# jhhung/kISS

Measured on AMD Instinct MI355X. Metric: bases/sec suffix_sort (chm13v2.0-size synthetic, k=256), higher is better.
Workload: dtype u8; 1 GPU; suffix_sort genome-like synthetic n=3117292070 k=256 (stand-in for chm13v2.0.fa, BASELINE.json configs[1]); PARALLEL_SORTING; text resident in HBM, SA left in HBM; n=3117292070, k=256, seed=2, parallelism=single GPU, lms=905939973, lms_rounds=9, tied_after_round0_item_rounds=184319413, big_segment_item_rounds=72866550, workspace_bytes=80356032300, induce_passes=47

## Files before the change

### include/kiss_hip.h

```cpp
#ifndef KISS_HIP_H
#define KISS_HIP_H

#include <stddef.h>
#include <stdint.h>

#ifdef __cplusplus
extern "C" {
#endif

#define KISS_HIP_VERSION 103

typedef enum kiss_hip_status {
    KISS_HIP_OK = 0,
    KISS_HIP_E_INVALID = -1,
    KISS_HIP_E_NO_DEVICE = -2,
    KISS_HIP_E_HIP = -3,
    KISS_HIP_E_NOMEM = -4,
    KISS_HIP_E_UNSUPPORTED = -5,
    KISS_HIP_E_INTERNAL = -6,
    KISS_HIP_E_IO = -7,
    KISS_HIP_E_DEEP = -8
} kiss_hip_status;

#define KISS_HIP_ALGO_PARALLEL_SORTING 0
// ... 2 lines not shown
#define KISS_HIP_MAX_N 4294963200ull

typedef struct kiss_hip_ctx kiss_hip_ctx;

typedef struct kiss_hip_stats {
    uint64_t n;
    uint64_t m;
    uint32_t k;
    uint32_t depth;
    uint32_t lms_rounds;
    uint32_t induce_passes;
    uint64_t near_end;
    uint64_t sort_item_rounds;
    uint64_t big_item_rounds;
    float ms_total;
    float ms_pack;
    float ms_classify;
    float ms_lms_sort;
    float ms_place;
    float ms_induce;
    float ms_kernel[16];
    uint64_t launches_kernel[16];
    uint64_t items_kernel[16];
    uint64_t refine_items;
    uint32_t refine_depth;
    uint32_t doubling_rounds;
    float ms_refine;
    float ms_h2d;
    float ms_d2h;
    uint32_t refine_form;
    float ms_fm_range;
    float ms_fm_locate;
    uint32_t tie_run_retries;
    uint32_t reserved_tail_;
} kiss_hip_stats;

enum {
    KISS_HIP_K_PACK = 0,
    KISS_HIP_K_CLASSIFY = 1,
    KISS_HIP_K_RADIX_HIST = 2,
    KISS_HIP_K_RADIX_SCATTER = 3,
    KISS_HIP_K_SCAN = 4,
    KISS_HIP_K_KEYGATHER = 5,
    KISS_HIP_K_FLAG_COMPACT = 6,
    KISS_HIP_K_PLACE = 7,
    KISS_HIP_K_INDUCE_COUNT = 8,
    KISS_HIP_K_INDUCE_SCATTER = 9,
    KISS_HIP_K_INDUCE_SMALL = 10,
    KISS_HIP_K_FM_QUERY = 11,
    KISS_HIP_K_FM_BUILD = 12,
    KISS_HIP_K_SEGRANK = 13,
    KISS_HIP_K_GROUP_HEADS = 14,
    KISS_HIP_K_ISA = 15,
    KISS_HIP_K_NCLASSES = 16
};

int kiss_hip_version(void);
int kiss_hip_has_hooks(void);
const char *kiss_hip_strerror(int status);
int kiss_hip_device_count(int *count);

int kiss_hip_ctx_create(kiss_hip_ctx **out, int device, uint64_t max_n);
int kiss_hip_ctx_create_sized(kiss_hip_ctx **out, int device, uint64_t max_n, uint64_t lms_capacity);
int kiss_hip_ctx_destroy(kiss_hip_ctx *ctx);
int kiss_hip_ctx_set_profiling(kiss_hip_ctx *ctx, int enabled);
int kiss_hip_ctx_set_profiling_mask(kiss_hip_ctx *ctx, uint64_t class_mask);
int kiss_hip_last_hip_error(const kiss_hip_ctx *ctx, const char **msg);
// ... 264 lines not shown
```

### kiss_amd/_lib.py

```python
import ctypes
import os

_HERE = os.path.dirname(os.path.abspath(__file__))
LIB_PATH = os.path.join(_HERE, "libkiss_hip.so")
HOOKS_LIB_PATH = os.path.join(_HERE, "libkiss_hip_hooks.so")

KISS_HIP_OK = 0
KISS_HIP_E_INVALID, KISS_HIP_E_NO_DEVICE, KISS_HIP_E_HIP, KISS_HIP_E_NOMEM = -1, -2, -3, -4
KISS_HIP_E_UNSUPPORTED, KISS_HIP_E_INTERNAL, KISS_HIP_E_IO, KISS_HIP_E_DEEP = -5, -6, -7, -8
ALGO_PARALLEL_SORTING = 0
ALGO_PREFIX_DOUBLING = 1
MAX_N = 4294963200
VIEW_LOCAL_KEYS, VIEW_LOCAL_POS, VIEW_PART_KEYS, VIEW_PART_POS, VIEW_SORTED, VIEW_SORTED_CTX = range(6)

KERNEL_CLASSES = [
    "pack", "classify", "radix_hist", "radix_scatter", "scan", "keygather", "flag_compact",
    "place", "induce_count", "induce_scatter", "induce_small", "fm_query", "fm_build", "segrank",
    "group_heads", "isa",
]


class Stats(ctypes.Structure):
    _fields_ = [
        ("n", ctypes.c_uint64), ("m", ctypes.c_uint64), ("k", ctypes.c_uint32), ("depth", ctypes.c_uint32),
        ("lms_rounds", ctypes.c_uint32), ("induce_passes", ctypes.c_uint32), ("near_end", ctypes.c_uint64),
        ("sort_item_rounds", ctypes.c_uint64), ("big_item_rounds", ctypes.c_uint64),
        ("ms_total", ctypes.c_float), ("ms_pack", ctypes.c_float), ("ms_classify", ctypes.c_float),
        ("ms_lms_sort", ctypes.c_float), ("ms_place", ctypes.c_float), ("ms_induce", ctypes.c_float),
        ("ms_kernel", ctypes.c_float * 16), ("launches_kernel", ctypes.c_uint64 * 16),
        ("items_kernel", ctypes.c_uint64 * 16),
        ("refine_items", ctypes.c_uint64), ("refine_depth", ctypes.c_uint32), ("doubling_rounds", ctypes.c_uint32),
        ("ms_refine", ctypes.c_float), ("ms_h2d", ctypes.c_float), ("ms_d2h", ctypes.c_float),
        ("refine_form", ctypes.c_uint32), ("ms_fm_range", ctypes.c_float), ("ms_fm_locate", ctypes.c_float),
        ("tie_run_retries", ctypes.c_uint32), ("reserved_tail_", ctypes.c_uint32),
    ]

    def as_dict(self):
        d = {k: getattr(self, k) for k, _ in self._fields_ if not k.endswith("_kernel")}
        d["kernels"] = {
            name: {"ms": self.ms_kernel[i], "launches": self.launches_kernel[i], "items": self.items_kernel[i]}
            for i, name in enumerate(KERNEL_CLASSES)
        }
        return d


class MultiStats(ctypes.Structure):
    _fields_ = [
        ("n", ctypes.c_uint64), ("m", ctypes.c_uint64), ("ndev", ctypes.c_uint32), ("refine_depth", ctypes.c_uint32),
        ("piece", ctypes.c_uint64 * 8),
        ("ms_total", ctypes.c_float), ("ms_pack", ctypes.c_float), ("ms_classify", ctypes.c_float),
        ("ms_partition", ctypes.c_float), ("ms_exchange", ctypes.c_float), ("ms_sort", ctypes.c_float),
        ("ms_gather", ctypes.c_float), ("ms_induce", ctypes.c_float),
    ]

    def as_dict(self):
        d = {k: getattr(self, k) for k, _ in self._fields_ if k != "piece"}
        d["piece"] = [int(x) for x in self.piece][:max(1, min(8, self.ndev))]
        return d


class VerifyReport(ctypes.Structure):
    _fields_ = [
        ("n", ctypes.c_uint64), ("k", ctypes.c_uint32), ("exact", ctypes.c_uint32), ("ok", ctypes.c_uint32),
        ("sa0_ok", ctypes.c_uint32), ("out_of_range", ctypes.c_uint64), ("duplicates", ctypes.c_uint64),
        ("order_violations", ctypes.c_uint64), ("first_violation", ctypes.c_uint64), ("tied_pairs", ctypes.c_uint64),
        ("digest", ctypes.c_uint64), ("ms", ctypes.c_float), ("reserved_", ctypes.c_uint32),
    ]
# ... 284 lines not shown
```

### kiss_amd/csrc/api.hip

```cpp
#include "kiss_internal.hpp"
#include <cstdlib>
#include <chrono>
#include <mutex>
#include <cstring>
#include <new>

KTimer::KTimer(kiss_hip_ctx *c, int cls, uint64_t items) : ctx(c), idx(-1)
{
    if (!((ctx->profile_mask >> cls) & 1ull)) return;
    if (ctx->ev_used == ctx->ev_pool.size()) {
        kiss_hip_ctx::Ev e;
        if (hipEventCreate(&e.a) != hipSuccess || hipEventCreate(&e.b) != hipSuccess) return;
        e.cls = 0;
        ctx->ev_pool.push_back(e);
    }
    idx = (int)ctx->ev_used++;
    ctx->ev_pool[idx].cls = cls;
    ctx->stats.launches_kernel[cls]++;
    ctx->stats.items_kernel[cls] += items;
    (void)hipEventRecord(ctx->ev_pool[idx].a, ctx->stream);
}
KTimer::~KTimer()
{
    if (idx >= 0) (void)hipEventRecord(ctx->ev_pool[idx].b, ctx->stream);
// ... 4 lines not shown
        float ms = 0.f;
        if (hipEventElapsedTime(&ms, ctx->ev_pool[i].a, ctx->ev_pool[i].b) == hipSuccess)
            ctx->stats.ms_kernel[ctx->ev_pool[i].cls] += ms;
    }
    ctx->ev_used = 0;
}

static void kiss_opts_supported_from_env(KissOpts &o)
{
    o.debug = getenv("KISS_HIP_DEBUG") != nullptr;
    if (const char *e = getenv("KISS_HIP_XFER_THREADS")) o.xfer_threads = atoi(e);
    if (const char *e = getenv("KISS_HIP_PREFAULT_THREADS")) o.prefault_threads = atoi(e);
}
#ifdef KISS_HIP_HOOKS
static bool env_on(const char *name) { return getenv(name) != nullptr; }
static unsigned long long env_u64(const char *name, unsigned long long dflt)
{
    const char *e = getenv(name);
    return e ? strtoull(e, nullptr, 0) : dflt;
}
void kiss_opts_refresh(kiss_hip_ctx *ctx)
{
    KissOpts o;
    kiss_opts_supported_from_env(o);
    if (const char *e = getenv("KISS_HIP_SYNC_READBACK")) o.sync_readback = atoi(e) != 0;
    o.no_serialize = env_on("KISS_HIP_NO_SERIALIZE");
    o.no_lms_exact = env_on("KISS_HIP_NO_LMS_EXACT");
    o.heads_by_compare = env_on("KISS_HIP_LMS_HEADS_BY_COMPARE");
    o.no_early_out = env_on("KISS_HIP_NO_EARLY_OUT");
    o.no_pivot_rounds = env_on("KISS_HIP_NO_PIVOT_ROUNDS");
    o.pivot_from_round2 = env_on("KISS_HIP_PIVOT_FROM_ROUND2");
    o.pair_keys = env_on("KISS_HIP_PAIR_KEYS");
    o.no_fc0_onepass = env_on("KISS_HIP_NO_FC0_ONEPASS");
    o.no_class_bytes = env_on("KISS_HIP_NO_CLASS_BYTES");
    o.no_pivot_ctx = env_on("KISS_HIP_NO_PIVOT_CTX");
    o.no_taint = env_on("KISS_HIP_NO_TAINT");
    o.isa_direct = env_on("KISS_HIP_ISA_DIRECT");
    o.no_onesweep = env_on("KISS_HIP_NO_ONESWEEP");
    o.rx_one_tile = env_on("KISS_HIP_RX_ONE_TILE");
    o.merge_lms = env_on("KISS_HIP_MERGE_LMS");
    o.no_small_alphabet = env_on("KISS_HIP_NO_SMALL_ALPHABET");
    o.induce_one_pass = env_on("KISS_HIP_INDUCE_ONE_PASS");
    o.verify = env_on("KISS_HIP_VERIFY");
    o.no_prefault = env_on("KISS_HIP_NO_PREFAULT");
    o.doubling_h0 = (uint32_t)env_u64("KISS_HIP_DOUBLING_H0", 0);
    o.tcap0 = env_u64("KISS_HIP_TCAP0", 0);
    o.pivot_slots = (int)env_u64("KISS_HIP_PIVOT_SLOTS", 3);
    o.small_seg = (uint32_t)env_u64("KISS_HIP_SMALL_SEG", 0);
    o.near_merge_min = (uint32_t)env_u64("KISS_HIP_NEAR_MERGE_MIN", 4096);
    o.induce_small_max = (uint32_t)env_u64("KISS_HIP_INDUCE_SMALL_MAX", 0);
    o.collapse_cap = (uint32_t)env_u64("KISS_HIP_COLLAPSE_CAP", 0);
    o.collapse_n = env_u64("KISS_HIP_COLLAPSE_N", 0);
    o.fm_heavy = (uint32_t)env_u64("KISS_HIP_FM_HEAVY", 0);
    o.fm_light = (uint32_t)env_u64("KISS_HIP_FM_LIGHT", 0);
    o.fm_mm_wave = env_on("KISS_HIP_FM_MM_WAVE");
    o.fm_mm_budget = env_u64("KISS_HIP_FM_MM_BUDGET", 0);
    o.fm8_group = env_on("KISS_HIP_FM8_GROUP");
    o.isa_direct_max = env_u64("KISS_HIP_ISA_DIRECT_MAX", 0);
    o.lx_sync_points = (unsigned)env_u64("KISS_HIP_LX_SYNC_POINTS", 0);
    o.tie_trace = (unsigned)env_u64("KISS_HIP_TIE_TRACE", 0);
    o.poison = (uint32_t)env_u64("KISS_HIP_POISON", 0);
    if (const char *e = getenv("KISS_HIP_DUMP_PIVOT")) snprintf(o.dump_pivot, sizeof o.dump_pivot, "%s", e);
    ctx->opts = o;
}
static std::mutex &kiss_launch_mutex()
{
// ... 302 lines not shown
{
    const bool dbg = ctx->opts.debug;
    const auto t_begin = std::chrono::steady_clock::now();
    free_lms_side(ctx);
    if (dbg)
        fprintf(stderr, "[kiss_hip] lms_reserve(%llu): freed the old arrays in %.3f s\n", (unsigned long long)m_cap,
                std::chrono::duration<double>(std::chrono::steady_clock::now() - t_begin).count());
    const uint64_t before = ctx->ws_bytes;
    ctx->m_cap = m_cap;
    const uint64_t radix_tiles = m_cap / 2048 + 2;
    ctx->tile_hist_cap = 256 * radix_tiles + 256 * (radix_tiles / 64 + 2) + 8;
    uint64_t biggest_scan = m_cap;
    if (ctx->tile_hist_cap > biggest_scan) biggest_scan = ctx->tile_hist_cap;
    if (ctx->ind_tiles_cap > biggest_scan) biggest_scan = ctx->ind_tiles_cap;
    if (ctx->n_tiles_cap > biggest_scan) biggest_scan = ctx->n_tiles_cap;
    ctx->scan_tmp_cap = biggest_scan / 4096 + 16;
    int rc = KISS_HIP_OK;
    do {
#define ALLOC(p, cnt) if ((rc = dmalloc(ctx, &ctx->p, (cnt)))) break
        ALLOC(lms_pos, m_cap);
        ALLOC(keyA, m_cap);
        ALLOC(keyB, m_cap);
        ALLOC(posA, m_cap);
        ALLOC(posB, m_cap);
        ALLOC(lms_sorted_far, m_cap);
        ALLOC(lms_ctx_far, m_cap);
        ALLOC(lmsP, m_cap);
        ALLOC(lmsC, m_cap);
        ALLOC(tile_hist, ctx->tile_hist_cap);
        ALLOC(scan_tmp, ctx->scan_tmp_cap);
        ctx->rx_tiles_cap = m_cap / 16384 + 2;
        ALLOC(rx_desc, 256 * ctx->rx_tiles_cap);
        ALLOC(rx_ghist, 256 * 12);
        ctx->fc_desc_cap = m_cap / 8192 + 4;
        ALLOC(fc_desc, ctx->fc_desc_cap);
#undef ALLOC
        if (hipMemset(ctx->rx_desc, 0, 256 * ctx->rx_tiles_cap * sizeof(uint64_t)) != hipSuccess) rc = KISS_HIP_E_HIP;
    } while (0);
    ctx->lms_bytes = ctx->ws_bytes - before;
    if (rc) {
        free_lms_side(ctx);
        ctx->m_cap = 0;
        return rc;
    }
    uint64_t t0 = m_cap / 4 + (4ull << 20);
    if (t0 > m_cap) t0 = m_cap;
    if (t_cap_wanted > t0) t0 = t_cap_wanted;
    if (ctx->opts.tcap0 >= 1 && ctx->opts.tcap0 < t0) t0 = ctx->opts.tcap0;
    if (dbg)
        fprintf(stderr, "[kiss_hip] lms_reserve(%llu): %.1f GB allocated, %.3f s so far\n", (unsigned long long)m_cap,
                (double)ctx->lms_bytes / 1e9, std::chrono::duration<double>(std::chrono::steady_clock::now() - t_begin).count());
    return kiss_tied_reserve(ctx, t0);
}

int kiss_tied_reserve(kiss_hip_ctx *ctx, uint64_t t_cap)
{
    const bool dbg = ctx->opts.debug;
    const auto t_begin = std::chrono::steady_clock::now();
    free_tied(ctx);
    const auto t_freed = std::chrono::steady_clock::now();
    if (t_cap < 1024) t_cap = 1024;
    const uint64_t before = ctx->ws_bytes;
    uint64_t fcap = 2 * t_cap;
    const uint64_t tiles_m = 2 * (ctx->m_cap / 2048 + 2), tiles_n = 2 * ((ctx->max_n + 1) / 2048 + 2);
    if (fcap < tiles_m) fcap = tiles_m;
    if (fcap < tiles_n) fcap = tiles_n;
    int rc = KISS_HIP_OK;
// ... 460 lines not shown
```

### kiss_amd/csrc/kiss_internal.hpp

```cpp
#pragma once
#include <hip/hip_runtime.h>
#include <stdint.h>
#include <stddef.h>
#include <mutex>
#include <vector>
#include "../../include/kiss_hip.h"

struct KissOpts {
    bool debug = false;
    int xfer_threads = 0;
    int prefault_threads = 0;
    bool sync_readback = false;
    bool no_lms_exact = false;
    bool heads_by_compare = false;
    bool no_early_out = false;
    bool no_pivot_rounds = false;
    bool pivot_from_round2 = false;
    bool pair_keys = false;
    bool no_fc0_onepass = false;
    bool no_class_bytes = false;
    bool no_pivot_ctx = false;
    bool no_taint = false;
    bool isa_direct = false;
    bool no_onesweep = false;
    bool rx_one_tile = false;
    bool merge_lms = false;
    bool no_small_alphabet = false;
    bool induce_one_pass = false;
    bool verify = false;
    bool no_prefault = false;
    bool no_serialize = false;
    bool lock_launches = false;
    bool sync_launches = false;
    uint32_t doubling_h0 = 0;
    uint64_t tcap0 = 0;
    int pivot_slots = 3;
    uint32_t small_seg = 0;
    uint32_t near_merge_min = 4096;
    uint32_t induce_small_max = 0;
    uint32_t collapse_cap = 0;
    uint64_t collapse_n = 0;
    uint32_t fm_heavy = 0, fm_light = 0;
    bool fm_mm_wave = false;
    bool fm8_group = false;
    uint64_t fm_mm_budget = 0;
    uint64_t isa_direct_max = 0;
    unsigned lx_sync_points = 0;
    unsigned tie_trace = 0;
    uint32_t poison = 0;
    char dump_pivot[256] = {0};
};
struct kiss_hip_ctx;
// ... 271 lines not shown
```

### kiss_amd/csrc/lms_sort.hip

```cpp
#include "kiss_internal.hpp"
#include <cstdio>
#include <cstdlib>
#include <cstring>
#include <ctime>
#include <utility>
#include <vector>

namespace {

constexpr int LS_THREADS = 256;
constexpr uint32_t SMALL_SEG = 64;
constexpr uint32_t LMS_SMALL_SEG = 24;
constexpr int ROUND0_BASES = 20;

__global__ __launch_bounds__(LS_THREADS) void k_gather_keys(const uint64_t *__restrict__ pk, uint64_t n,
                                                           const uint32_t *__restrict__ pos, uint64_t count,
                                                           uint64_t depth_off, uint64_t mask,
                                                           uint64_t *__restrict__ key, const uint32_t *__restrict__ seg,
                                                           const uint32_t *__restrict__ segstart, uint32_t min_len,
                                                           uint32_t max_len)
{
    uint64_t i = (uint64_t)blockIdx.x * LS_THREADS + threadIdx.x;
    if (i >= count) return;
    if (seg) {
// ... 133 lines not shown
                    if (j == (uint32_t)i) continue;
                    uint64_t kj = key[j];
                    bool jless;
                    if (kj != ki) jless = kj < ki;
                    else {
                        bool tj = false;
                        jless = deep_less(pk, n, pos[j], pi, off, depth, j < (uint32_t)i, &tj);
                        taint = taint || tj;
                        tied_before = tied_before || (tj && jless);
                    }
                    r += jless ? 1u : 0u;
                }
            }
        }
    }
    const uint32_t r_prev = __shfl_up(r, 1, 64);
    const bool t_prev = __shfl_up((int)taint, 1, 64) != 0;
    if (second_in_wave) {
        r = 1u - r_prev;
        taint = t_prev;
    }
    if (small && b - a == 2) tied_before = taint && r == 1;
    if (small) {
        const uint32_t dst = slot[a + r];
        out[dst] = (uint32_t)pi;
        if (hfar && tied_before) hfar[dst] = 0;
        if (tctx) octx[dst] = tctx[i] | (taint ? KISS_CTX_TAINT : 0u);
        else if (taint) octx[dst] = KISS_CTX_TAINT;
        big[i] = 0;
    } else if (valid) {
        big[i] = (uint32_t)i == a ? (uint8_t)3 : (uint8_t)1;
    }
    (void)nbig;
}

__device__ __forceinline__ uint32_t pivot_class(const uint64_t *__restrict__ bkey, uint32_t a, uint32_t b, uint64_t k)
{
    const uint64_t pv = bkey[(a + b) >> 1];
    return k < pv ? 0u : (k == pv ? 1u : 2u);
}

__global__ __launch_bounds__(LS_THREADS) void k_pivot_class(const uint64_t *__restrict__ bkey,
                                                           const uint32_t *__restrict__ bseg,
                                                           const uint32_t *__restrict__ bsegstart, uint64_t nbig,
                                                           uint64_t *__restrict__ cls)
{
    const uint64_t i = (uint64_t)blockIdx.x * LS_THREADS + threadIdx.x;
    if (i >= nbig) return;
    const uint32_t sid = bseg[i];
    const uint32_t c = pivot_class(bkey, bsegstart[sid], bsegstart[sid + 1], bkey[i]);
    cls[i] = c == 0 ? 1ull : (c == 1 ? (1ull << 32) : 0ull);
}

__global__ __launch_bounds__(LS_THREADS) void k_pivot_scatter(const uint64_t *__restrict__ bkey,
                                                             const uint32_t *__restrict__ bpos,
                                                             const uint32_t *__restrict__ bseg,
                                                             const uint32_t *__restrict__ bsegstart, uint64_t nbig,
                                                             const uint64_t *__restrict__ cls,
                                                             const uint64_t *__restrict__ ex,
                                                             const uint64_t *__restrict__ tot,
                                                             uint64_t *__restrict__ okey, uint32_t *__restrict__ opos,
                                                             uint64_t *__restrict__ ne)
{
    const uint64_t i = (uint64_t)blockIdx.x * LS_THREADS + threadIdx.x;
    if (i >= nbig) return;
    const uint32_t sid = bseg[i];
// ... 461 lines not shown
#define KISS_FC1_MIN_WAVES 1
#endif
#ifndef KISS_FC1_STORE_UNROLL
#define KISS_FC1_STORE_UNROLL 4
#endif
constexpr int FC1_THREADS = KISS_FC1_THREADS;
constexpr int FC1_ITEMS = KISS_FC1_ITEMS;
constexpr int FC1_CHUNKS = FC1_ITEMS / 2;
constexpr int FC1_WAVE_ITEMS = 64 * FC1_ITEMS;
constexpr int FC1_TILE = FC1_THREADS * FC1_ITEMS;
constexpr uint32_t FC1_SPIN_LIMIT = 1u << 22;
static_assert(FC1_ITEMS % 2 == 0 && FC1_ITEMS <= 16, "two items per lane and chunk; four flag bits per chunk in one word");

#ifdef FC_PROF
__device__ unsigned long long fc_prof[12];
#define FC_MARK(i)                                                                                                     \
    do {                                                                                                               \
        if (threadIdx.x == 0) {                                                                                        \
            const unsigned long long now_ = wall_clock64();                                                            \
            atomicAdd(&fc_prof[i], now_ - t_prev_);                                                                    \
            t_prev_ = now_;                                                                                            \
        }                                                                                                              \
    } while (0)
#else
#define FC_MARK(i)
#endif
__device__ __forceinline__ uint64_t lane_value_u64(uint64_t v, int src_lane)
{
    const uint32_t lo = (uint32_t)__builtin_amdgcn_readlane((int)(uint32_t)v, src_lane);
    const uint32_t hi = (uint32_t)__builtin_amdgcn_readlane((int)(uint32_t)(v >> 32), src_lane);
    return ((uint64_t)hi << 32) | lo;
}

__global__ __launch_bounds__(FC1_THREADS, KISS_FC1_MIN_WAVES) void k_fc0_onepass(const uint64_t *__restrict__ key,
                                                            const uint32_t *__restrict__ pos, uint64_t count,
                                                            int cmp_shift, uint64_t tiles, uint64_t *__restrict__ desc,
                                                            uint32_t *__restrict__ ticket, uint32_t *__restrict__ err,
                                                            uint32_t *__restrict__ npos, uint32_t *__restrict__ nslot,
                                                            uint32_t *__restrict__ nseg, uint32_t *__restrict__ nsegstart,
                                                            uint32_t *__restrict__ octx, uint32_t *__restrict__ nctx,
                                                            uint64_t cap, uint64_t *__restrict__ total)
{
    __shared__ uint32_t ws[FC1_THREADS / 64][2];
    __shared__ uint32_t s_tile;
    __shared__ uint32_t s_excl[2];
#ifdef FC_PROF
    unsigned long long t_prev_ = wall_clock64();
#endif
    if (threadIdx.x == 0) s_tile = atomicAdd(ticket, 1u);
    __syncthreads();
    FC_MARK(0);
    const uint64_t tile = s_tile;
    if (tile >= tiles) return;
    const int wave = threadIdx.x >> 6;
    const uint32_t lane = lane_id();
    const uint64_t wbase = tile * FC1_TILE + (uint64_t)wave * FC1_WAVE_ITEMS;
    const bool full = wbase + FC1_WAVE_ITEMS <= count;
    uint64_t k0[FC1_CHUNKS], k1[FC1_CHUNKS];
    uint32_t c0[FC1_CHUNKS], c1[FC1_CHUNKS];
#pragma unroll
    for (int j = 0; j < FC1_CHUNKS; j++) {
        const uint64_t a = wbase + (uint64_t)j * 128 + 2 * lane;
        ulonglong2 kk;
        if (full) kk = *reinterpret_cast<const ulonglong2 *>(key + a);
        else {
            kk.x = a < count ? key[a] : 0ull;
            kk.y = a + 1 < count ? key[a + 1] : 0ull;
        }
        k0[j] = kk.x >> cmp_shift;
        k1[j] = kk.y >> cmp_shift;
        c0[j] = (uint32_t)(kk.x & KISS_KEY_CTX_MASK);
        c1[j] = (uint32_t)(kk.y & KISS_KEY_CTX_MASK);
    }
    const bool has_prev = wbase > 0 && wbase < count, has_next = wbase + FC1_WAVE_ITEMS < count;
    const uint64_t kprev = has_prev ? key[wbase - 1] >> cmp_shift : 0ull;
    const uint64_t knext = has_next ? key[wbase + FC1_WAVE_ITEMS] >> cmp_shift : 0ull;
    uint32_t p0[FC1_CHUNKS], p1[FC1_CHUNKS];
#pragma unroll
    for (int j = 0; j < FC1_CHUNKS; j++) {
        const uint64_t a = wbase + (uint64_t)j * 128 + 2 * lane;
        if (full) {
            const uint2 t = *reinterpret_cast<const uint2 *>(pos + a);
            p0[j] = t.x;
            p1[j] = t.y;
        } else {
            p0[j] = a < count ? pos[a] : 0u;
            p1[j] = a + 1 < count ? pos[a + 1] : 0u;
        }
    }
#ifdef FC_PROF
    asm volatile("s_waitcnt vmcnt(0)" ::: "memory");
    FC_MARK(1);
#endif
    uint64_t H0[FC1_CHUNKS];
    uint32_t h01 = 0;
#pragma unroll
    for (int j = 0; j < FC1_CHUNKS; j++) {
        const uint64_t a = wbase + (uint64_t)j * 128 + 2 * lane;
        uint64_t up = __shfl_up(k1[j], 1, 64);
        const uint64_t before = j == 0 ? kprev : lane_value_u64(k1[j > 0 ? j - 1 : 0], 63);
        if (lane == 0) up = before;
        const bool h0 = a == 0 || a >= count || up != k0[j];
        const bool h1 = a + 1 >= count || k0[j] != k1[j];
        H0[j] = __ballot(h0);
        h01 |= (h0 ? 1u : 0u) << (2 * j) | (h1 ? 1u : 0u) << (2 * j + 1);
    }
    const bool next_head = !has_next || lane_value_u64(k1[FC1_CHUNKS - 1], 63) != knext;
    uint32_t fl = 0;
    uint32_t rs[FC1_CHUNKS], gs[FC1_CHUNKS];
    uint32_t run_s = 0, run_h = 0;
    const uint64_t below = (1ull << lane) - 1ull;
#pragma unroll
    for (int j = 0; j < FC1_CHUNKS; j++) {
        const uint64_t a = wbase + (uint64_t)j * 128 + 2 * lane;
        const bool h0 = (h01 >> (2 * j)) & 1u, h1 = (h01 >> (2 * j + 1)) & 1u;
        const uint64_t nxt = j + 1 < FC1_CHUNKS ? H0[j + 1 < FC1_CHUNKS ? j + 1 : j] : (next_head ? 1ull : 0ull);
        const bool hn = lane < 63u ? ((H0[j] >> (lane + 1u)) & 1ull) != 0 : (nxt & 1ull) != 0;
        const bool s0 = a < count && !(h0 && h1), s1 = a + 1 < count && !(h1 && hn);
        const bool m0 = s0 && h0, m1 = s1 && h1;
        const uint64_t S0 = __ballot(s0), S1 = __ballot(s1), M0 = __ballot(m0), M1 = __ballot(m1);
        rs[j] = run_s + (uint32_t)__popcll(S0 & below) + (uint32_t)__popcll(S1 & below);
        gs[j] = run_h + (uint32_t)__popcll(M0 & below) + (uint32_t)__popcll(M1 & below);
        run_s += (uint32_t)__popcll(S0) + (uint32_t)__popcll(S1);
        run_h += (uint32_t)__popcll(M0) + (uint32_t)__popcll(M1);
        fl |= ((s0 ? 1u : 0u) | (s1 ? 2u : 0u) | (m0 ? 4u : 0u) | (m1 ? 8u : 0u)) << (4 * j);
    }
    if (lane == 0) {
        ws[wave][0] = run_s;
        ws[wave][1] = run_h;
    }
    FC_MARK(2);
    __syncthreads();
    FC_MARK(3);
    uint32_t ts = 0, th = 0, ws0 = 0, wh0 = 0;
#pragma unroll
    for (int w = 0; w < FC1_THREADS / 64; w++) {
        if (w < wave) {
            ws0 += ws[w][0];
            wh0 += ws[w][1];
        }
        ts += ws[w][0];
        th += ws[w][1];
    }
    if (wave == 0) {
        constexpr uint64_t M31 = 0x7FFFFFFFull;
        const uint64_t mine = ((uint64_t)ts << 31) | (uint64_t)th;
        uint64_t es = 0, eh = 0;
        if (tile == 0) {
            if (lane == 0) __hip_atomic_store(&desc[0], (2ull << 62) | mine, __ATOMIC_RELAXED, __HIP_MEMORY_SCOPE_AGENT);
        } else {
            if (lane == 0) __hip_atomic_store(&desc[tile], (1ull << 62) | mine, __ATOMIC_RELAXED, __HIP_MEMORY_SCOPE_AGENT);
            int64_t base = (int64_t)tile;
            uint32_t spins = 0;
            for (;;) {
                const int64_t t = base - 1 - (int64_t)lane;
                const uint64_t v = t >= 0 ? __hip_atomic_load(&desc[t], __ATOMIC_RELAXED, __HIP_MEMORY_SCOPE_AGENT)
                                          : (2ull << 62);
                const uint32_t st = (uint32_t)(v >> 62);
                const uint64_t incl = __ballot(st == 2u), ready = __ballot(st != 0u);
                const uint32_t first = incl ? (uint32_t)__builtin_ctzll(incl) : 64u;
                const uint64_t need = first >= 63u ? ~0ull : ((2ull << first) - 1ull);
                if ((ready & need) != need) {
                    if (++spins > FC1_SPIN_LIMIT) {
                        if (lane == 0) *err = 1;
                        break;
                    }
                    __builtin_amdgcn_s_sleep(1);
                    continue;
                }
                uint64_t a = lane <= first ? (v >> 31) & M31 : 0ull, b = lane <= first ? v & M31 : 0ull;
#pragma unroll
                for (int d = 32; d >= 1; d >>= 1) {
                    a += __shfl_xor(a, d, 64);
                    b += __shfl_xor(b, d, 64);
                }
                es += a;
                eh += b;
                if (first < 64u) break;
                base -= 64;
            }
            if (lane == 0)
                __hip_atomic_store(&desc[tile], (2ull << 62) | ((es + ts) << 31) | (eh + th), __ATOMIC_RELAXED,
                                   __HIP_MEMORY_SCOPE_AGENT);
        }
        if (lane == 0) {
            s_excl[0] = (uint32_t)es;
            s_excl[1] = (uint32_t)eh;
            if (tile + 1 == tiles) total[0] = ((es + ts) << 32) | (eh + th);
        }
    }
    FC_MARK(4);
    __syncthreads();
    FC_MARK(5);
    if (wbase >= count) return;
    const uint32_t bs = s_excl[0] + ws0, bh = s_excl[1] + wh0;
#pragma unroll KISS_FC1_STORE_UNROLL
    for (int j = 0; j < FC1_CHUNKS; j++) {
        const uint64_t a = wbase + (uint64_t)j * 128 + 2 * lane;
        const uint32_t f = (fl >> (4 * j)) & 15u;
        const uint32_t ni0 = bs + rs[j], ni1 = ni0 + (f & 1u);
        const uint32_t sid0 = bh + gs[j] + ((f >> 2) & 1u) - 1u;
        const uint32_t sid1 = sid0 + ((f >> 3) & 1u);
        if (f & 1u) {
            if (ni0 < cap) {
                npos[ni0] = p0[j];
                nslot[ni0] = (uint32_t)a;
                nseg[ni0] = sid0;
                if (f & 4u) nsegstart[sid0] = ni0;
                if (nctx) nctx[ni0] = c0[j];
            }
            c0[j] = 0;
        }
        if (f & 2u) {
            if (ni1 < cap) {
                npos[ni1] = p1[j];
                nslot[ni1] = (uint32_t)(a + 1);
                nseg[ni1] = sid1;
                if (f & 8u) nsegstart[sid1] = ni1;
                if (nctx) nctx[ni1] = c1[j];
            }
            c1[j] = 0;
        }
        if (full) *reinterpret_cast<uint2 *>(octx + a) = make_uint2(c0[j], c1[j]);
        else {
            if (a < count) octx[a] = c0[j];
            if (a + 1 < count) octx[a + 1] = c1[j];
        }
    }
    FC_MARK(6);
#ifdef FC_PROF
    asm volatile("s_waitcnt vmcnt(0)" ::: "memory");
    FC_MARK(7);
#endif
}

__device__ __forceinline__ void fch_flags(const uint8_t *__restrict__ hb, uint64_t i0, uint64_t count, uint32_t &valid,
                                          uint32_t &survmask, uint32_t &headmask)
{
    valid = i0 >= count ? 0u : (count - i0 >= FC_ITEMS ? (uint32_t)FC_ITEMS : (uint32_t)(count - i0));
    survmask = headmask = 0;
    if (!valid) return;
    uint8_t h[FC_ITEMS + 1];
    if (valid == FC_ITEMS) {
        const uint64_t w = *reinterpret_cast<const uint64_t *>(hb + i0);
#pragma unroll
        for (int e = 0; e < FC_ITEMS; e++) h[e] = (uint8_t)(w >> (8 * e));
    } else {
#pragma unroll
        for (int e = 0; e < FC_ITEMS; e++) h[e] = (uint32_t)e < valid ? hb[i0 + e] : (uint8_t)1;
    }
    h[FC_ITEMS] = i0 + FC_ITEMS < count ? hb[i0 + FC_ITEMS] : (uint8_t)1;
#pragma unroll
    for (int e = 0; e < FC_ITEMS; e++) {
        if ((uint32_t)e < valid) {
            const uint64_t i = i0 + (uint64_t)e;
            const bool head = i == 0 || h[e] != 0;
            const bool nhead = i + 1 == count || h[e + 1] != 0;
            const bool surv = !(head && nhead);
            survmask |= (surv ? 1u : 0u) << e;
// ... 262 lines not shown
        *p = v;
        if (zero_me) *zero_me = 0;
    }
}

int bits_for(uint64_t count)
{
    int b = 0;
    if (count > 1) {
        uint64_t v = count - 1;
        while (v) {
            b++;
            v >>= 1;
        }
    }
    return b;
}

int read_u64(kiss_hip_ctx *ctx, const void *dptr, uint64_t *out)
{
    KTRY(kiss_readback(ctx, dptr, 2));
    std::memcpy(out, ctx->h_pinned, sizeof(uint64_t));
    return KISS_HIP_OK;
}

}

int kiss_lms_sort(kiss_hip_ctx *ctx, uint64_t n, uint32_t k, uint64_t depth)
{
    (void)k;
    const uint64_t m_far = ctx->m_far;
    ctx->stats.lms_rounds = 0;
    ctx->stats.sort_item_rounds = 0;
    if (m_far == 0) return KISS_HIP_OK;
    if (m_far == 1) {
        KCHECK(hipMemcpyAsync(ctx->lms_sorted_far, ctx->lms_pos, sizeof(uint32_t), hipMemcpyDeviceToDevice,
                              ctx->stream));
        KTRY(kiss_zero_u32(ctx, ctx->lms_ctx_far, 1));
        return KISS_HIP_OK;
    }
    uint32_t *d_nbig = ctx->d_small + 8;
    uint64_t *d_total = (uint64_t *)(ctx->d_small + 2);
    const unsigned T = LS_THREADS;
    const bool dbg = ctx->opts.debug;
    const bool pivot_on = !ctx->opts.no_pivot_rounds;
    const bool pivot_r1 = !ctx->opts.pivot_from_round2;
    static const int pivot_den[3] = {4, 7, 11};
    unsigned pivot_rounds_done = 0;
    const int pivot_slots = ctx->opts.pivot_slots >= 1 && ctx->opts.pivot_slots <= 8 ? ctx->opts.pivot_slots : 3;
    const bool no_pair_keys = !ctx->opts.pair_keys;
    const uint32_t small_seg = ctx->opts.small_seg >= 2 && ctx->opts.small_seg <= 4096 ? ctx->opts.small_seg : LMS_SMALL_SEG;

    uint64_t count = m_far;
    RadixBufs rb;
    rb.first_pos = ctx->lms_pos;
    rb.key[0] = ctx->keyA;
    rb.key[1] = ctx->keyB;
    rb.pos[0] = ctx->posA;
    static_assert(KISS_R0_PASSES % 2 == 1, "round-0 result must land in buffer 1");
    rb.pos[1] = ctx->lms_sorted_far;
    rb.seg[0] = rb.seg[1] = nullptr;
    const int r0_shift = 64 - 2 * ROUND0_BASES;
    static_assert(64 - 2 * ROUND0_BASES == KISS_R0_SHIFT && (2 * ROUND0_BASES + 7) / 8 == KISS_R0_PASSES, "classify.hip counts these digits");
    int res = 0;
    KTRY(kiss_radix_sort(ctx, rb, count, r0_shift, 0, &res));
    ctx->stats.lms_rounds++;
    ctx->stats.sort_item_rounds += count;
    uint32_t *Pc = rb.pos[res ^ 1];
    uint64_t tot;
    bool have_tctx = false;
    const bool no_onepass = ctx->opts.no_fc0_onepass;
    const uint64_t tiles1 = div_up(count, FC1_TILE);
    const bool onepass = !no_onepass && ctx->fc_desc && tiles1 >= 8 && tiles1 + 1 <= ctx->fc_desc_cap &&
                         rb.pos[res] == ctx->lms_sorted_far;
    if (onepass) {
        uint64_t *desc = ctx->fc_desc;
        uint32_t *ticket = reinterpret_cast<uint32_t *>(desc + tiles1);
        for (int attempt = 0; attempt < 2; attempt++) {
            KTRY(kiss_zero_u32(ctx, desc, 2 * tiles1 + 2));
            {
                KTimer t(ctx, KISS_HIP_K_FLAG_COMPACT, count);
                hipLaunchKernelGGL(k_fc0_onepass, dim3((unsigned)tiles1), dim3(FC1_THREADS), 0, ctx->stream, rb.key[res], rb.pos[res],
                                   count, r0_shift, tiles1, desc, ticket, ctx->rx_ctl + 1, Pc, ctx->slotA, ctx->segA, ctx->segstartA,
                                   ctx->lms_ctx_far, ctx->bslot, ctx->t_cap, d_total);
                KCHECK(hipGetLastError());
            }
            KTRY(fc_read_total(ctx, d_total, &tot));
#ifdef FC_PROF
            {
                unsigned long long h[12], z[12] = {0};
                KCHECK(hipMemcpyFromSymbol(h, HIP_SYMBOL(fc_prof), sizeof h));
                KCHECK(hipMemcpyToSymbol(HIP_SYMBOL(fc_prof), z, sizeof z));
                unsigned long long sum = 0;
                for (int i = 0; i < 8; i++) sum += h[i];
                fprintf(stderr, "[fc_prof] %llu tiles, %.2f us per tile (100 MHz clock):", (unsigned long long)tiles1, (double)sum / 100.0 / (double)tiles1);
                for (int i = 0; i < 8; i++) fprintf(stderr, " %d:%.1f%%", i, sum ? 100.0 * (double)h[i] / (double)sum : 0.0);
                fprintf(stderr, "\n");
            }
#endif
            if ((tot >> 32) <= ctx->t_cap) break;
            if (attempt) return KINTERNAL();
            const uint64_t surv = tot >> 32;
            KTRY(kiss_tied_reserve(ctx, surv + surv / 8 + 1024));
        }
        have_tctx = true;
    } else {
        KTRY((fc_count<FC_KEY>(ctx, rb.key[res], nullptr, count, r0_shift, 0, d_total)));
        KTRY(fc_read_total(ctx, d_total, &tot));
        if ((tot >> 32) > ctx->t_cap) {
            const uint64_t surv = tot >> 32;
            KTRY(kiss_tied_reserve(ctx, surv + surv / 8 + 1024));
            KTRY((fc_count<FC_KEY>(ctx, rb.key[res], nullptr, count, r0_shift, 0, d_total)));
        }
    }
    uint32_t *Sc = ctx->slotA, *Gc = ctx->segA, *SSc = ctx->segstartA;
    uint64_t *F1 = ctx->flags;
    uint64_t *F2 = ctx->flags + ctx->t_cap;
    if (!onepass)
        KTRY((fc_compact<FC_KEY, false>(ctx, rb.key[res], nullptr, rb.pos[res], nullptr, count, r0_shift, 0, Pc, Sc, Gc, SSc,
                                       ctx->lms_sorted_far, nullptr, ctx->lms_ctx_far, ctx->bslot, &have_tctx)));
    count = tot >> 32;
    uint64_t nseg = tot & 0xFFFFFFFFull;
    if (dbg)
        fprintf(stderr, "[kiss_hip] round 0: items %llu -> survivors %llu in %llu segments\n",
                (unsigned long long)m_far, (unsigned long long)count, (unsigned long long)nseg);
    uint64_t *K1 = ctx->keyA;

    uint64_t off = ROUND0_BASES;
    bool first_refine = true;
    for (;; first_refine = false) {
        if (count == 0) break;
        if (depth && off >= depth) return KINTERNAL();
        uint64_t rem = depth ? depth - off : 32;
        if (rem > 32) rem = 32;
        const bool last_round = depth ? (off + 32 >= depth) : false;
        const uint64_t mask = rem >= 32 ? ~0ull : (~0ull << (64 - 2 * rem));
        const int key_lo_bit = (int)(64 - 2 * rem);
        const unsigned grid = (unsigned)div_up(count, T);
        const bool pivot_ahead = depth && (off > ROUND0_BASES || pivot_r1) && pivot_on;
        {
            KTimer t(ctx, KISS_HIP_K_KEYGATHER, count);
            hipLaunchKernelGGL(k_set_u32, dim3(1), dim3(64), 0, ctx->stream, SSc + nseg, (uint32_t)count, (uint32_t *)nullptr);
            hipLaunchKernelGGL(k_gather_keys, dim3(grid), dim3(T), 0, ctx->stream, ctx->pk, n, Pc, count, off, mask,
                               K1, no_pair_keys ? Gc : (const uint32_t *)nullptr, SSc, 3u, pivot_ahead ? small_seg : 0xFFFFFFFFu);
            KCHECK(hipGetLastError());
        }
        uint8_t *bigb = nullptr;
        hipEvent_t dbg_e0 = nullptr, dbg_e1 = nullptr;
        if (dbg) {
            (void)hipEventCreate(&dbg_e0);
            (void)hipEventCreate(&dbg_e1);
            (void)hipEventRecord(dbg_e0, ctx->stream);
        }
        {
            KTimer t(ctx, KISS_HIP_K_SEGRANK, count);
            hipLaunchKernelGGL(k_set_u32, dim3(1), dim3(64), 0, ctx->stream, SSc + nseg, (uint32_t)count, d_nbig);
            uint8_t *inorder = reinterpret_cast<uint8_t *>(F2);
            bigb = inorder + ((count + 15) & ~15ull);
            hipLaunchKernelGGL(k_seg_adjacent, dim3(grid), dim3(T), 0, ctx->stream, ctx->pk, n, K1, Pc, Gc, SSc, count, off,
                               depth, small_seg, inorder);
            hipLaunchKernelGGL(k_seg_finish, dim3(grid), dim3(T), 0, ctx->stream, ctx->pk, n, K1, Pc, Sc, Gc, SSc,
// ... 1032 lines not shown
```

Baseline: 42.84 billion bases/s.

## Resolve size-2 tied segments after round 0 with a direct pair compare kernel

The round-0 one-pass flag-compact kernel now detects tie segments of exactly two items. It leaves them out of the survivor set and writes pair records (two positions plus an output slot) into a spare buffer, with a second decoupled-lookback prefix for the record count. A new k_pair_finish kernel then resolves each pair with a deep string comparison, swaps the pair if needed and propagates taint context. This keeps pairs out of the iterative key-gather/radix refinement rounds. In exchange it adds shuffle-based head-flag computation in place of ballots, a doubled lookback descriptor array, and an extra 10-bit packed rank field.

New measurement: 44.16 billion bases/s (median of 6 runs). 1.03x the previous value.

```diff
diff --git a/include/kiss_hip.h b/include/kiss_hip.h
--- a/include/kiss_hip.h
+++ b/include/kiss_hip.h
@@ -58,7 +58,7 @@
     float ms_fm_range;
     float ms_fm_locate;
     uint32_t tie_run_retries;
-    uint32_t reserved_tail_;
+    uint32_t pair_records;
 } kiss_hip_stats;
 
 enum {
diff --git a/kiss_amd/_lib.py b/kiss_amd/_lib.py
--- a/kiss_amd/_lib.py
+++ b/kiss_amd/_lib.py
@@ -32,7 +32,7 @@
         ("refine_items", ctypes.c_uint64), ("refine_depth", ctypes.c_uint32), ("doubling_rounds", ctypes.c_uint32),
         ("ms_refine", ctypes.c_float), ("ms_h2d", ctypes.c_float), ("ms_d2h", ctypes.c_float),
         ("refine_form", ctypes.c_uint32), ("ms_fm_range", ctypes.c_float), ("ms_fm_locate", ctypes.c_float),
-        ("tie_run_retries", ctypes.c_uint32), ("reserved_tail_", ctypes.c_uint32),
+        ("tie_run_retries", ctypes.c_uint32), ("pair_records", ctypes.c_uint32),
     ]
 
     def as_dict(self):
diff --git a/kiss_amd/csrc/api.hip b/kiss_amd/csrc/api.hip
--- a/kiss_amd/csrc/api.hip
+++ b/kiss_amd/csrc/api.hip
@@ -60,6 +60,7 @@
     o.pivot_from_round2 = env_on("KISS_HIP_PIVOT_FROM_ROUND2");
     o.pair_keys = env_on("KISS_HIP_PAIR_KEYS");
     o.no_fc0_onepass = env_on("KISS_HIP_NO_FC0_ONEPASS");
+    o.no_pair_records = env_on("KISS_HIP_NO_PAIR_RECORDS");
     o.no_class_bytes = env_on("KISS_HIP_NO_CLASS_BYTES");
     o.no_pivot_ctx = env_on("KISS_HIP_NO_PIVOT_CTX");
     o.no_taint = env_on("KISS_HIP_NO_TAINT");
@@ -428,7 +429,7 @@
         ctx->rx_tiles_cap = m_cap / 16384 + 2;
         ALLOC(rx_desc, 256 * ctx->rx_tiles_cap);
         ALLOC(rx_ghist, 256 * 12);
-        ctx->fc_desc_cap = m_cap / 8192 + 4;
+        ctx->fc_desc_cap = 2 * (m_cap / 8192 + 4);
         ALLOC(fc_desc, ctx->fc_desc_cap);
 #undef ALLOC
         if (hipMemset(ctx->rx_desc, 0, 256 * ctx->rx_tiles_cap * sizeof(uint64_t)) != hipSuccess) rc = KISS_HIP_E_HIP;
diff --git a/kiss_amd/csrc/kiss_internal.hpp b/kiss_amd/csrc/kiss_internal.hpp
--- a/kiss_amd/csrc/kiss_internal.hpp
+++ b/kiss_amd/csrc/kiss_internal.hpp
@@ -18,6 +18,7 @@
     bool pivot_from_round2 = false;
     bool pair_keys = false;
     bool no_fc0_onepass = false;
+    bool no_pair_records = false;
     bool no_class_bytes = false;
     bool no_pivot_ctx = false;
     bool no_taint = false;
diff --git a/kiss_amd/csrc/lms_sort.hip b/kiss_amd/csrc/lms_sort.hip
--- a/kiss_amd/csrc/lms_sort.hip
+++ b/kiss_amd/csrc/lms_sort.hip
@@ -189,6 +189,30 @@
         big[i] = (uint32_t)i == a ? (uint8_t)3 : (uint8_t)1;
     }
     (void)nbig;
+}
+
+__global__ __launch_bounds__(LS_THREADS) void k_pair_finish(const uint64_t *__restrict__ pk, uint64_t n,
+                                                           const uint32_t *__restrict__ rpos0,
+                                                           const uint32_t *__restrict__ rpos1,
+                                                           const uint32_t *__restrict__ rslot, uint64_t npairs,
+                                                           uint64_t off, uint64_t depth, uint32_t *__restrict__ out,
+                                                           uint32_t *__restrict__ octx, uint8_t *__restrict__ hfar)
+{
+    const uint64_t i = (uint64_t)blockIdx.x * LS_THREADS + threadIdx.x;
+    if (i >= npairs) return;
+    const uint32_t p0 = rpos0[i], p1 = rpos1[i], s = rslot[i];
+    bool taint = false;
+    const bool swap = deep_less(pk, n, p1, p0, off - 32, depth, false, &taint);
+    if (!swap && !taint) return;
+    const uint32_t c0 = octx[s], c1 = octx[s + 1];
+    const uint32_t t = taint ? KISS_CTX_TAINT : 0u;
+    if (swap) {
+        out[s] = p1;
+        out[s + 1] = p0;
+    }
+    octx[s] = (swap ? c1 : c0) | t;
+    octx[s + 1] = (swap ? c0 : c1) | t;
+    if (hfar && taint) hfar[s + 1] = 0;
 }
 
 __device__ __forceinline__ uint32_t pivot_class(const uint64_t *__restrict__ bkey, uint32_t a, uint32_t b, uint64_t k)
@@ -716,6 +740,7 @@
     return ((uint64_t)hi << 32) | lo;
 }
 
+template <bool PAIRS>
 __global__ __launch_bounds__(FC1_THREADS, KISS_FC1_MIN_WAVES) void k_fc0_onepass(const uint64_t *__restrict__ key,
                                                             const uint32_t *__restrict__ pos, uint64_t count,
                                                             int cmp_shift, uint64_t tiles, uint64_t *__restrict__ desc,
@@ -723,11 +748,13 @@
                                                             uint32_t *__restrict__ npos, uint32_t *__restrict__ nslot,
                                                             uint32_t *__restrict__ nseg, uint32_t *__restrict__ nsegstart,
                                                             uint32_t *__restrict__ octx, uint32_t *__restrict__ nctx,
-                                                            uint64_t cap, uint64_t *__restrict__ total)
-{
-    __shared__ uint32_t ws[FC1_THREADS / 64][2];
+                                                            uint64_t cap, uint64_t *__restrict__ total,
+                                                            uint32_t *__restrict__ rec, uint32_t rcol)
+{
+    constexpr int DS = PAIRS ? 2 : 1;
+    __shared__ uint32_t ws[FC1_THREADS / 64][3];
     __shared__ uint32_t s_tile;
-    __shared__ uint32_t s_excl[2];
+    __shared__ uint32_t s_excl[3];
 #ifdef FC_PROF
     unsigned long long t_prev_ = wall_clock64();
 #endif
@@ -776,7 +803,6 @@
     asm volatile("s_waitcnt vmcnt(0)" ::: "memory");
     FC_MARK(1);
 #endif
-    uint64_t H0[FC1_CHUNKS];
     uint32_t h01 = 0;
 #pragma unroll
     for (int j = 0; j < FC1_CHUNKS; j++) {
@@ -786,61 +812,94 @@
         if (lane == 0) up = before;
         const bool h0 = a == 0 || a >= count || up != k0[j];
         const bool h1 = a + 1 >= count || k0[j] != k1[j];
-        H0[j] = __ballot(h0);
         h01 |= (h0 ? 1u : 0u) << (2 * j) | (h1 ? 1u : 0u) << (2 * j + 1);
     }
+    const uint32_t h01_up = __shfl_down(h01, 1, 64);
+    const uint32_t h01_l0 = (uint32_t)__builtin_amdgcn_readlane((int)h01, 0);
     const bool next_head = !has_next || lane_value_u64(k1[FC1_CHUNKS - 1], 63) != knext;
     uint32_t fl = 0;
-    uint32_t rs[FC1_CHUNKS], gs[FC1_CHUNKS];
-    uint32_t run_s = 0, run_h = 0;
+    uint32_t rk[FC1_CHUNKS];
+    static_assert(FC1_WAVE_ITEMS < 1024, "rank fields of 10 bits");
+    uint32_t run_s = 0, run_h = 0, run_p = 0;
+    uint32_t pair_carry = 0;
     const uint64_t below = (1ull << lane) - 1ull;
 #pragma unroll
     for (int j = 0; j < FC1_CHUNKS; j++) {
-        const uint64_t a = wbase + (uint64_t)j * 128 + 2 * lane;
-        const bool h0 = (h01 >> (2 * j)) & 1u, h1 = (h01 >> (2 * j + 1)) & 1u;
-        const uint64_t nxt = j + 1 < FC1_CHUNKS ? H0[j + 1 < FC1_CHUNKS ? j + 1 : j] : (next_head ? 1ull : 0ull);
-        const bool hn = lane < 63u ? ((H0[j] >> (lane + 1u)) & 1ull) != 0 : (nxt & 1ull) != 0;
-        const bool s0 = a < count && !(h0 && h1), s1 = a + 1 < count && !(h1 && hn);
-        const bool m0 = s0 && h0, m1 = s1 && h1;
-        const uint64_t S0 = __ballot(s0), S1 = __ballot(s1), M0 = __ballot(m0), M1 = __ballot(m1);
-        rs[j] = run_s + (uint32_t)__popcll(S0 & below) + (uint32_t)__popcll(S1 & below);
-        gs[j] = run_h + (uint32_t)__popcll(M0 & below) + (uint32_t)__popcll(M1 & below);
+        const uint32_t h0 = (h01 >> (2 * j)) & 1u, h1 = (h01 >> (2 * j + 1)) & 1u;
+        const uint32_t nb = lane < 63u ? h01_up >> (2 * j) : (j + 1 < FC1_CHUNKS ? h01_l0 >> (2 * j + 2) : (next_head ? 1u : 0u));
+        const uint32_t hn = nb & 1u;
+        uint32_t s0 = (h0 & h1) ^ 1u, s1 = (h1 & hn) ^ 1u;
+        if (PAIRS) {
+            const uint32_t hnn = (nb >> 1) & 1u;
+            const uint32_t pf0 = h0 & (h1 ^ 1u) & hn;
+            const uint32_t pf1 = h1 & (hn ^ 1u) & hnn;
+            uint32_t ps0 = __shfl_up(pf1, 1, 64);
+            if (lane == 0u) ps0 = pair_carry;
+            pair_carry = (uint32_t)__builtin_amdgcn_readlane((int)pf1, 63);
+            s0 &= (pf0 | ps0) ^ 1u;
+            s1 &= (pf1 | pf0) ^ 1u;
+            const uint64_t PF = __ballot((pf0 | pf1) != 0u);
+            rk[j] = (run_p + (uint32_t)__popcll(PF & below)) << 20;
+            run_p += (uint32_t)__popcll(PF);
+            fl |= (pf0 | (pf1 << 1)) << (16 + 2 * j);
+        }
+        const uint32_t m0 = s0 & h0, m1 = s1 & h1;
+        const uint64_t S0 = __ballot(s0 != 0u), S1 = __ballot(s1 != 0u), M0 = __ballot(m0 != 0u), M1 = __ballot(m1 != 0u);
+        if (!PAIRS) rk[j] = 0;
+        rk[j] |= run_s + (uint32_t)__popcll(S0 & below) + (uint32_t)__popcll(S1 & below);
+        rk[j] |= (run_h + (uint32_t)__popcll(M0 & below) + (uint32_t)__popcll(M1 & below)) << 10;
         run_s += (uint32_t)__popcll(S0) + (uint32_t)__popcll(S1);
         run_h += (uint32_t)__popcll(M0) + (uint32_t)__popcll(M1);
-        fl |= ((s0 ? 1u : 0u) | (s1 ? 2u : 0u) | (m0 ? 4u : 0u) | (m1 ? 8u : 0u)) << (4 * j);
+        fl |= (s0 | (s1 << 1) | (m0 << 2) | (m1 << 3)) << (4 * j);
     }
     if (lane == 0) {
         ws[wave][0] = run_s;
         ws[wave][1] = run_h;
+        ws[wave][2] = run_p;
     }
     FC_MARK(2);
     __syncthreads();
     FC_MARK(3);
-    uint32_t ts = 0, th = 0, ws0 = 0, wh0 = 0;
+    uint32_t ts = 0, th = 0, tp = 0, ws0 = 0, wh0 = 0, wp0 = 0;
 #pragma unroll
     for (int w = 0; w < FC1_THREADS / 64; w++) {
         if (w < wave) {
             ws0 += ws[w][0];
             wh0 += ws[w][1];
+            if (PAIRS) wp0 += ws[w][2];
         }
         ts += ws[w][0];
         th += ws[w][1];
+        if (PAIRS) tp += ws[w][2];
     }
     if (wave == 0) {
         constexpr uint64_t M31 = 0x7FFFFFFFull;
         const uint64_t mine = ((uint64_t)ts << 31) | (uint64_t)th;
-        uint64_t es = 0, eh = 0;
+        constexpr uint64_t M62 = (1ull << 62) - 1ull;
+        uint64_t es = 0, eh = 0, ep = 0;
         if (tile == 0) {
-            if (lane == 0) __hip_atomic_store(&desc[0], (2ull << 62) | mine, __ATOMIC_RELAXED, __HIP_MEMORY_SCOPE_AGENT);
+            if (lane == 0) {
+                __hip_atomic_store(&desc[0], (2ull << 62) | mine, __ATOMIC_RELAXED, __HIP_MEMORY_SCOPE_AGENT);
+                if (PAIRS) __hip_atomic_store(&desc[1], (2ull << 62) | (uint64_t)tp, __ATOMIC_RELAXED, __HIP_MEMORY_SCOPE_AGENT);
+            }
         } else {
-            if (lane == 0) __hip_atomic_store(&desc[tile], (1ull << 62) | mine, __ATOMIC_RELAXED, __HIP_MEMORY_SCOPE_AGENT);
+            if (lane == 0) {
+                __hip_atomic_store(&desc[DS * tile], (1ull << 62) | mine, __ATOMIC_RELAXED, __HIP_MEMORY_SCOPE_AGENT);
+                if (PAIRS)
+                    __hip_atomic_store(&desc[DS * tile + 1], (1ull << 62) | (uint64_t)tp, __ATOMIC_RELAXED, __HIP_MEMORY_SCOPE_AGENT);
+            }
             int64_t base = (int64_t)tile;
             uint32_t spins = 0;
             for (;;) {
                 const int64_t t = base - 1 - (int64_t)lane;
-                const uint64_t v = t >= 0 ? __hip_atomic_load(&desc[t], __ATOMIC_RELAXED, __HIP_MEMORY_SCOPE_AGENT)
+                const uint64_t v = t >= 0 ? __hip_atomic_load(&desc[DS * t], __ATOMIC_RELAXED, __HIP_MEMORY_SCOPE_AGENT)
                                           : (2ull << 62);
-                const uint32_t st = (uint32_t)(v >> 62);
+                uint32_t st = (uint32_t)(v >> 62);
+                uint64_t v2 = 0;
+                if (PAIRS) {
+                    v2 = t >= 0 ? __hip_atomic_load(&desc[DS * t + 1], __ATOMIC_RELAXED, __HIP_MEMORY_SCOPE_AGENT) : (2ull << 62);
+                    if ((uint32_t)(v2 >> 62) != st) st = 0;
+                }
                 const uint64_t incl = __ballot(st == 2u), ready = __ballot(st != 0u);
                 const uint32_t first = incl ? (uint32_t)__builtin_ctzll(incl) : 64u;
                 const uint64_t need = first >= 63u ? ~0ull : ((2ull << first) - 1ull);
@@ -853,37 +912,49 @@
                     continue;
                 }
                 uint64_t a = lane <= first ? (v >> 31) & M31 : 0ull, b = lane <= first ? v & M31 : 0ull;
+                uint64_t c = lane <= first ? v2 & M62 : 0ull;
 #pragma unroll
                 for (int d = 32; d >= 1; d >>= 1) {
                     a += __shfl_xor(a, d, 64);
                     b += __shfl_xor(b, d, 64);
+                    if (PAIRS) c += __shfl_xor(c, d, 64);
                 }
                 es += a;
                 eh += b;
+                ep += c;
                 if (first < 64u) break;
                 base -= 64;
             }
-            if (lane == 0)
-                __hip_atomic_store(&desc[tile], (2ull << 62) | ((es + ts) << 31) | (eh + th), __ATOMIC_RELAXED,
+            if (lane == 0) {
+                __hip_atomic_store(&desc[DS * tile], (2ull << 62) | ((es + ts) << 31) | (eh + th), __ATOMIC_RELAXED,
                                    __HIP_MEMORY_SCOPE_AGENT);
+                if (PAIRS)
+                    __hip_atomic_store(&desc[DS * tile + 1], (2ull << 62) | (ep + tp), __ATOMIC_RELAXED, __HIP_MEMORY_SCOPE_AGENT);
+            }
         }
         if (lane == 0) {
             s_excl[0] = (uint32_t)es;
             s_excl[1] = (uint32_t)eh;
-            if (tile + 1 == tiles) total[0] = ((es + ts) << 32) | (eh + th);
+            s_excl[2] = (uint32_t)ep;
+            if (tile + 1 == tiles) {
+                total[0] = ((es + ts) << 32) | (eh + th);
+                total[1] = ep + tp;
+            }
         }
     }
     FC_MARK(4);
     __syncthreads();
     FC_MARK(5);
     if (wbase >= count) return;
-    const uint32_t bs = s_excl[0] + ws0, bh = s_excl[1] + wh0;
+    const uint32_t bs = s_excl[0] + ws0, bh = s_excl[1] + wh0, bp = s_excl[2] + wp0;
+    uint32_t lane_st = lane;
+    asm volatile("" : "+v"(lane_st));
 #pragma unroll KISS_FC1_STORE_UNROLL
     for (int j = 0; j < FC1_CHUNKS; j++) {
-        const uint64_t a = wbase + (uint64_t)j * 128 + 2 * lane;
+        const uint64_t a = wbase + (uint64_t)j * 128 + 2 * lane_st;
         const uint32_t f = (fl >> (4 * j)) & 15u;
-        const uint32_t ni0 = bs + rs[j], ni1 = ni0 + (f & 1u);
-        const uint32_t sid0 = bh + gs[j] + ((f >> 2) & 1u) - 1u;
+        const uint32_t ni0 = bs + (rk[j] & 1023u), ni1 = ni0 + (f & 1u);
+        const uint32_t sid0 = bh + ((rk[j] >> 10) & 1023u) + ((f >> 2) & 1u) - 1u;
         const uint32_t sid1 = sid0 + ((f >> 3) & 1u);
         if (f & 1u) {
             if (ni0 < cap) {
@@ -909,6 +980,24 @@
         else {
             if (a < count) octx[a] = c0[j];
             if (a + 1 < count) octx[a + 1] = c1[j];
+        }
+    }
+    if (PAIRS) {
+#pragma unroll
+        for (int j = 0; j < FC1_CHUNKS; j++) {
+            const uint32_t a32 = (uint32_t)wbase + (uint32_t)j * 128u + 2u * lane_st;
+            const uint32_t pf = (fl >> (16 + 2 * j)) & 3u;
+            uint32_t pn = __shfl_down(p0[j], 1, 64);
+            if (j + 1 < FC1_CHUNKS) {
+                const uint32_t w0 = (uint32_t)__builtin_amdgcn_readlane((int)p0[j + 1 < FC1_CHUNKS ? j + 1 : j], 0);
+                if (lane == 63u) pn = w0;
+            }
+            if (pf) {
+                const uint32_t ri = bp + (rk[j] >> 20);
+                rec[ri] = (pf & 1u) ? p0[j] : p1[j];
+                rec[rcol + ri] = (pf & 1u) ? p1[j] : pn;
+                rec[2u * rcol + ri] = a32 + (pf >> 1);
+            }
         }
     }
     FC_MARK(6);
@@ -1237,6 +1326,7 @@
     const uint64_t m_far = ctx->m_far;
     ctx->stats.lms_rounds = 0;
     ctx->stats.sort_item_rounds = 0;
+    ctx->stats.pair_records = 0;
     if (m_far == 0) return KISS_HIP_OK;
     if (m_far == 1) {
         KCHECK(hipMemcpyAsync(ctx->lms_sorted_far, ctx->lms_pos, sizeof(uint32_t), hipMemcpyDeviceToDevice,
@@ -1276,21 +1366,32 @@
     bool have_tctx = false;
     const bool no_onepass = ctx->opts.no_fc0_onepass;
     const uint64_t tiles1 = div_up(count, FC1_TILE);
-    const bool onepass = !no_onepass && ctx->fc_desc && tiles1 >= 8 && tiles1 + 1 <= ctx->fc_desc_cap &&
+    const bool onepass = !no_onepass && ctx->fc_desc && tiles1 >= 8 && 2 * tiles1 + 1 <= ctx->fc_desc_cap &&
                          rb.pos[res] == ctx->lms_sorted_far;
+    const bool pair_records = onepass && !ctx->opts.no_pair_records && rb.key[res] == ctx->keyB;
+    const uint64_t rcol = (count / 2 + 4) & ~3ull;
+    uint32_t *const rpos0 = reinterpret_cast<uint32_t *>(ctx->keyA), *const rpos1 = rpos0 + rcol, *const rslot = rpos1 + rcol;
+    uint64_t npairs = 0;
     if (onepass) {
         uint64_t *desc = ctx->fc_desc;
-        uint32_t *ticket = reinterpret_cast<uint32_t *>(desc + tiles1);
+        uint32_t *ticket = reinterpret_cast<uint32_t *>(desc + 2 * tiles1);
         for (int attempt = 0; attempt < 2; attempt++) {
-            KTRY(kiss_zero_u32(ctx, desc, 2 * tiles1 + 2));
+            KTRY(kiss_zero_u32(ctx, desc, 4 * tiles1 + 2));
             {
                 KTimer t(ctx, KISS_HIP_K_FLAG_COMPACT, count);
-                hipLaunchKernelGGL(k_fc0_onepass, dim3((unsigned)tiles1), dim3(FC1_THREADS), 0, ctx->stream, rb.key[res], rb.pos[res],
-                                   count, r0_shift, tiles1, desc, ticket, ctx->rx_ctl + 1, Pc, ctx->slotA, ctx->segA, ctx->segstartA,
-                                   ctx->lms_ctx_far, ctx->bslot, ctx->t_cap, d_total);
+                if (pair_records)
+                    hipLaunchKernelGGL(k_fc0_onepass<true>, dim3((unsigned)tiles1), dim3(FC1_THREADS), 0, ctx->stream, rb.key[res],
+                                       rb.pos[res], count, r0_shift, tiles1, desc, ticket, ctx->rx_ctl + 1, Pc, ctx->slotA, ctx->segA,
+                                       ctx->segstartA, ctx->lms_ctx_far, ctx->bslot, ctx->t_cap, d_total, rpos0, (uint32_t)rcol);
+                else
+                    hipLaunchKernelGGL(k_fc0_onepass<false>, dim3((unsigned)tiles1), dim3(FC1_THREADS), 0, ctx->stream, rb.key[res],
+                                       rb.pos[res], count, r0_shift, tiles1, desc, ticket, ctx->rx_ctl + 1, Pc, ctx->slotA, ctx->segA,
+                                       ctx->segstartA, ctx->lms_ctx_far, ctx->bslot, ctx->t_cap, d_total, (uint32_t *)nullptr, 0u);
                 KCHECK(hipGetLastError());
             }
-            KTRY(fc_read_total(ctx, d_total, &tot));
+            KTRY(kiss_readback(ctx, d_total, 4));
+            std::memcpy(&tot, ctx->h_pinned, sizeof(uint64_t));
+            std::memcpy(&npairs, ctx->h_pinned + 2, sizeof(uint64_t));
 #ifdef FC_PROF
             {
                 unsigned long long h[12], z[12] = {0};
@@ -1309,6 +1410,14 @@
             KTRY(kiss_tied_reserve(ctx, surv + surv / 8 + 1024));
         }
         have_tctx = true;
+        if (npairs) {
+            if (npairs > count / 2) return KINTERNAL();
+            KTimer t(ctx, KISS_HIP_K_SEGRANK, 2 * npairs);
+            hipLaunchKernelGGL(k_pair_finish, dim3((unsigned)div_up(npairs, T)), dim3(T), 0, ctx->stream, ctx->pk, n, rpos0, rpos1,
+                               rslot, npairs, (uint64_t)ROUND0_BASES, depth, ctx->lms_sorted_far, ctx->lms_ctx_far, ctx->hfar);
+            KCHECK(hipGetLastError());
+            ctx->stats.pair_records = (uint32_t)npairs;
+        }
     } else {
         KTRY((fc_count<FC_KEY>(ctx, rb.key[res], nullptr, count, r0_shift, 0, d_total)));
         KTRY(fc_read_total(ctx, d_total, &tot));
@@ -1332,6 +1441,10 @@
     uint64_t *K1 = ctx->keyA;
 
     uint64_t off = ROUND0_BASES;
+    if (npairs) {
+        ctx->stats.sort_item_rounds += 2 * npairs;
+        if (count == 0) ctx->stats.lms_rounds++;
+    }
     bool first_refine = true;
     for (;; first_refine = false) {
         if (count == 0) break;
```
